# WesleyHsieh0806/TAO-Amodal

Measured on AMD Instinct MI355X. Metric: box-pair IoU+match throughput, higher is better.
Workload: dtype f64

## Files before the change

### include/tao_amodal_hip.h

```cpp
#ifndef TAO_AMODAL_HIP_H
#define TAO_AMODAL_HIP_H

#include <stddef.h>
#include <stdint.h>

#ifdef __cplusplus
extern "C" {
#endif

#define TAOAMD_N_THR 10
#define TAOAMD_N_REC 101
#define TAOAMD_LVIS_RNG 6
#define TAOAMD_TAO_RNG 20

#define TAOAMD_GT_IGNORE 1
#define TAOAMD_GT_OOF 2
#define TAOAMD_GT_ID_HIDDEN 4
#define TAOAMD_DT_IGNORE_UNMATCHED 1
#define TAOAMD_DT_NO_CONSUME 2

#define TAOAMD_OK 0
#define TAOAMD_ERR_HIP 1
#define TAOAMD_ERR_ARG 2
#define TAOAMD_ERR_TOO_LARGE 3
// ... 6 lines not shown

int taoamd_kernel_timing_enable(int on);
int taoamd_kernel_timing_label(const char *label);
int taoamd_kernel_timing_collect(char *names_host, size_t names_bytes,
                                 double *total_ms_host, int64_t *calls_host,
                                 int32_t max_kernels, int32_t *n_kernels_host);

int taoamd_thresholds_host(double *iou_thrs, double *rec_thrs);

int taoamd_set_thresholds(const double *iou_thrs, const double *rec_thrs);
int taoamd_set_ranges(const double *visibility_rng, const double *area_rng,
                      const double *time_rng);

int taoamd_bb_iou(const double *dt, const double *gt, size_t m, size_t n,
                  const unsigned char *iscrowd, double *o, void *stream);
int taoamd_bb_iou_host(const double *dt, const double *gt, size_t m, size_t n,
                       const unsigned char *iscrowd, double *o);

int taoamd_lvis_ranges(int64_t n_gt, const double *gt_vis,
                       const uint8_t *gt_flags, const int32_t *gt_cat,
                       const int32_t *gt_cat_off, int64_t n_dt,
                       const uint8_t *dt_flags, int32_t n_cat,
                       uint32_t *gt_rng, uint32_t *dt_rng, int32_t *num_gt,
                       void *stream);
int taoamd_tao_ranges(int64_t n_gt, const double *gt_area,
                      const int32_t *gt_len, const int32_t *gt_nhp,
                      const uint8_t *gt_flags, const int32_t *gt_cat,
                      const int32_t *gt_cat_off, int64_t n_dt,
                      const double *dt_area, const int32_t *dt_len,
                      const uint8_t *dt_flags, int32_t n_cat,
                      uint32_t *gt_rng, uint32_t *dt_rng, int32_t *num_gt,
                      void *stream);

size_t taoamd_rle_iou_workspace(int64_t n_dt, int64_t dt_total, int64_t n_gt,
                                int64_t gt_total);
int taoamd_rle_iou(int64_t n_cells, const int32_t *cell_dt_off,
                   const int32_t *cell_gt_off, const int64_t *cell_iou_off,
                   int64_t n_dt, int64_t dt_total, const int64_t *dt_off,
                   const uint32_t *dt_runs, const int32_t *dt_hw,
                   const double *dt_bb, int64_t n_gt, int64_t gt_total,
                   const int64_t *gt_off, const uint32_t *gt_runs,
                   const int32_t *gt_hw, const double *gt_bb, double *iou,
                   void *workspace, size_t workspace_bytes, void *stream);

size_t taoamd_track_mask_iou_workspace(int64_t dt_frames, int64_t dt_total,
                                       int64_t gt_frames, int64_t gt_total);
// ... 465 lines not shown
```

### tao_amodal_amd/_lib.py

```python
import ctypes as C
import os

HERE = os.path.dirname(os.path.abspath(__file__))
SO_PATH = os.environ.get("TAOAMD_LIBRARY") or os.path.join(HERE, "libtao_amodal_hip.so")

OK = 0
ERR_HIP, ERR_ARG, JSON_FALLBACK = 1, 2, 16
N_THR, N_REC = 10, 101
LVIS_RNG, TAO_RNG = 6, 20
MAX_GT_PER_CELL = 3072
SEGMENT_TILE = 2816
ERROR_TYPES_TILE = 256
TRACK_ERROR_TYPES_TILE = 16
ERROR_TYPES = ("TP", "IGNORED", "DUP", "LOC", "CLS", "BOTH", "BKG")
ERROR_IMPACT_CHUNK = 256
ERROR_FIXES = ("BASE", "CLS", "LOC", "BOTH", "DUP", "BKG", "MISS", "FP", "FN")
TRACK_ASSOCIATION_TILE = 64
TRACK_ASSOCIATION_VIS = 8
ASSOC_TRACK_COLUMNS = ("frames", "covered", "ids", "switches", "fragments", "primary",
                       "primary_frames")
ASSOC_CAT_COLUMNS = ("tracks", "frames", "covered", "ids", "switches", "fragments",
                     "mostly_tracked", "mostly_lost")
ASSOC_VIS_COLUMNS = ("frames", "covered", "primary")

_vp, _i64, _i32, _sz = C.c_void_p, C.c_int64, C.c_int32, C.c_size_t

SIGNATURES = {
    "taoamd_strerror": (C.c_char_p, [C.c_int]),
    "taoamd_last_error": (C.c_char_p, []),
    "taoamd_version": (C.c_int, []),
    "taoamd_thresholds_host": (C.c_int, [_vp, _vp]),
    "taoamd_set_thresholds": (C.c_int, [_vp, _vp]),
    "taoamd_set_ranges": (C.c_int, [_vp, _vp, _vp]),
    "taoamd_kernel_timing_enable": (C.c_int, [C.c_int]),
    "taoamd_kernel_timing_label": (C.c_int, [C.c_char_p]),
    "taoamd_kernel_timing_collect": (C.c_int, [_vp, _sz, _vp, _vp, _i32, _vp]),
    "taoamd_bb_iou": (C.c_int, [_vp, _vp, _sz, _sz, _vp, _vp, _vp]),
    "taoamd_bb_iou_host": (C.c_int, [_vp, _vp, _sz, _sz, _vp, _vp]),
    "taoamd_lvis_ranges": (C.c_int, [_i64, _vp, _vp, _vp, _vp, _i64, _vp,
                                     _i32, _vp, _vp, _vp, _vp]),
    "taoamd_tao_ranges": (C.c_int, [_i64, _vp, _vp, _vp, _vp, _vp, _vp, _i64,
                                    _vp, _vp, _vp, _i32, _vp, _vp, _vp, _vp]),
    "taoamd_sort_segments_workspace": (_sz, [_i64]),
    "taoamd_sort_segments": (C.c_int, [_i64, _i32, _vp, _vp, _i32, _i32, _vp,
                                       _vp, _vp, _vp, _vp, _sz, _vp]),
    "taoamd_sort_plan_host": (C.c_int, [_i32, _vp, _vp, _vp, _vp, _vp, _vp]),
    "taoamd_sort_sampled_workspace": (_sz, [_i64, _i64, _i32]),
    "taoamd_sort_sampled_cap_limit": (C.c_int, [_i32]),
    "taoamd_sort_sampled_notify": (C.c_int, [_vp]),
    "taoamd_event_create": (C.c_int, [_vp]),
    "taoamd_event_destroy": (C.c_int, [_vp]),
    "taoamd_stream_wait_event": (C.c_int, [_vp, _vp]),
    "taoamd_sort_sampled": (C.c_int, [_i64, _i32, _vp, _vp, _i32, _i32, _vp, _i32, _vp,
                                      _i32, _vp, _i32, _vp, _i32, _vp, _vp, _vp, _vp,
                                      _sz, _vp]),
    "taoamd_track_iou": (C.c_int, [_i64, _vp, _vp, _vp, _i64, _vp, _vp, _vp,
                                   _vp, _vp, _vp, _i32, _vp, _vp, _vp]),
    "taoamd_track_iou_single": (C.c_int, [_i64, _vp, _vp, _vp, _vp, _vp, _vp, _i32,
                                          _vp, _vp, _vp]),
    "taoamd_track_iou_planned": (C.c_int, [_i64, _vp, _vp, _vp, _vp, _vp, _vp, _vp,
                                           _i32, _vp, _vp, _i64, _vp, _vp]),
    "taoamd_track_stream": (C.c_int, [_i64, _vp, _vp, _vp, _vp, _vp, _vp, _vp]),
    "taoamd_json_pred_workspace": (_sz, [_sz]),
# ... 245 lines not shown
```

### tao_amodal_amd/csrc/accumulate.hip

```cpp
#include <atomic>
#include <cstdlib>
#include <cstring>

#include "common.hpp"
#include "transpose64.hpp"
#include "workspace.hpp"

using namespace taoamd;

#ifndef ACC_CH
#define ACC_CH 256
#endif
#ifndef ACC_INLINE_CHUNKS
#define ACC_INLINE_CHUNKS 64
#endif

struct AccArgs {
    int64_t n_dt;
    int32_t n_cat, n_rng, n_words, n_chunks_max;
    int32_t paired;
    int32_t wide;
    const int32_t *cat_off;
    const uint64_t *matched;
    const uint64_t *ignored;
// ... 1358 lines not shown
{
    AccArgs a;
    acc_layout(c, n_dt, n_cat, n_rng, a);
    val = c.take<double>(taoamd_compact_elems(n_cat, n_rng));
    rec = c.take<double>((size_t)n_cat * n_rng * N_THR);
}

extern "C" size_t taoamd_accumulate_workspace(int64_t n_dt, int32_t n_cat,
                                              int32_t n_rng)
{
    double *val, *rec;
    return measure([&](Carve &c) { acc_full_layout(c, n_dt, n_cat, n_rng, val, rec); });
}

enum { ACC_ALL = 0, ACC_PLAN = 1, ACC_SWEEP = 2 };

static int accumulate_compact(int64_t n_dt, int32_t n_cat, int32_t n_rng,
                              const int32_t *cat_off, const int32_t *order,
                              const uint64_t *matched, const uint64_t *ignored,
                              const int32_t *num_gt, int32_t k_begin, int32_t k_end,
                              int32_t max_segment, double *val, double *rec,
                              void *workspace, size_t workspace_bytes, void *stream,
                              int phase = ACC_ALL, int force_mode = SWEEP_AUTO,
                              const uint32_t *compact = nullptr)
{
    if (n_cat <= 0 || n_rng < 1 || n_rng > 32) return TAOAMD_ERR_ARG;
    if (k_begin < 0 || k_end > n_cat || k_begin > k_end) return TAOAMD_ERR_ARG;
    if (!cat_off || !workspace) return TAOAMD_ERR_ARG;
    if (phase != ACC_PLAN && (!num_gt || !val || !rec)) return TAOAMD_ERR_ARG;
    Carve c(workspace);
    AccArgs a;
    const AccWs t = acc_layout(c, n_dt, n_cat, n_rng, a);
    if (!c.fits(workspace, workspace_bytes)) return TAOAMD_ERR_WORKSPACE;
    if (k_begin == k_end) return TAOAMD_OK;
    hipStream_t s = (hipStream_t)stream;
    a.chunk_tab = nullptr;
    a.n_dt = n_dt; a.n_cat = n_cat; a.n_rng = n_rng;
    a.cat_off = cat_off; a.matched = matched; a.ignored = ignored; a.order = order;
    a.compact = compact;
    a.paired = matched != nullptr && ignored == matched + 1;
    a.wide = a.paired && ((uintptr_t)matched & 15) == 0;
    a.num_gt = num_gt; a.val = (uint64_t *)val; a.rec = rec;
    a.k_begin = k_begin; a.k_end = k_end;
    a.inline_scans = 0;
    a.sc_rows = 0; a.sc_gen = 0;
    a.sc_error = nullptr;
    a.sc_giveups = g_sweep_giveups.load(std::memory_order_relaxed);
// ... 35 lines not shown
    a.inline_scans = max_segment > 0 && max_segment <= ACC_INLINE_CHUNKS * ACC_CH;
    const size_t nc = (size_t)a.n_chunks_max, nw = (size_t)a.n_words;
    const int mode = force_mode != SWEEP_AUTO ? force_mode : sweep_mode(n_dt);
    if (compact != nullptr && (mode == SWEEP_CHUNKED || !order || !a.wide || a.n_words != 1 || n_rng > 6))
        return TAOAMD_ERR_ARG;
    if (mode != SWEEP_CHUNKED) {
        a.sc_rows = SWEEP_SW * SWEEP_NB * WAVE;
        a.inline_scans = 0;
    }
    if (mode != SWEEP_CHUNKED && max_segment > 0) a.xcd_start = t.xcd_start;
    if (phase == ACC_SWEEP) a.chunk_tab = t.chunk_tab;
    const unsigned chunk_blocks = (unsigned)((nc * nw + 3) / 4);
    const unsigned cat_blocks = (unsigned)((size_t)(k_end - k_begin) * nw);
    if (phase != ACC_SWEEP)
        TAO_TIMED("acc_chunks_kernel", s, acc_chunks_kernel<<<1, 256, 0, s>>>(a));
    if (phase == ACC_PLAN) {
        TAO_TIMED("acc_chunktab_kernel", s, acc_chunktab_kernel<<<(unsigned)((nc + 255) / 256), 256, 0, s>>>(a, t.chunk_tab));
        if (mode != SWEEP_CHUNKED)
            TAO_HIP(hipMemsetAsync(t.header, 0, t.head_bytes, s));
        TAO_LAUNCH_CHECK();
        return TAOAMD_OK;
    }
    if (mode != SWEEP_CHUNKED) {
        {
            const int64_t n_cj = (int64_t)n_cat * n_rng * N_REC;
            TAO_TIMED("acc_cj_kernel", s, acc_cj_kernel<<<(unsigned)((n_cj + 255) / 256), 256, 0, s>>>(a, rec_thr()));
        }
        const size_t n_sc = (size_t)(n_dt / a.sc_rows) + (size_t)n_cat + 1;
        const unsigned grid = a.xcd_start == nullptr
            ? (unsigned)(n_sc * nw)
            : (unsigned)(N_XCD * (n_sc / N_XCD + (size_t)max_segment / a.sc_rows + 3) * nw);
        if (mode == SWEEP_LOOKBACK) {
            if (phase == ACC_ALL)
                TAO_HIP(hipMemsetAsync(t.header, 0, t.head_bytes, s));
            uint32_t g = ++g_sc_gen;
            a.sc_gen = (g & 0x3fffffffu) ? (g & 0x3fffffffu) : (++g_sc_gen & 0x3fffffffu);
            a.sc_error = t.header;
            if (a.compact)
                TAO_TIMED("acc_sweep_kernel", s, (acc_sweep_kernel<SWEEP_SW, 0, 2><<<grid, SWEEP_SW * WAVE, 0, s>>>(a, rec_thr())));
            else if (a.order)
                TAO_TIMED("acc_sweep_kernel", s, (acc_sweep_kernel<SWEEP_SW, 0, 1><<<grid, SWEEP_SW * WAVE, 0, s>>>(a, rec_thr())));
            else
                TAO_TIMED("acc_sweep_kernel", s, (acc_sweep_kernel<SWEEP_SW, 0><<<grid, SWEEP_SW * WAVE, 0, s>>>(a, rec_thr())));
        } else if (a.compact) {
            TAO_TIMED("acc_sccount_kernel", s, (acc_sweep_kernel<SWEEP_SW, 2, 2><<<grid, SWEEP_SW * WAVE, 0, s>>>(a, rec_thr())));
            TAO_TIMED("acc_sweep_kernel", s, (acc_sweep_kernel<SWEEP_SW, 1, 2><<<grid, SWEEP_SW * WAVE, 0, s>>>(a, rec_thr())));
        } else if (a.order) {
// ... 15 lines not shown
    } else {
        TAO_TIMED("acc_prefix_kernel", s, acc_prefix_kernel<<<cat_blocks, 256, 0, s>>>(a, rec_thr()));
        TAO_TIMED("acc_chunkmax_kernel", s, acc_chunkmax_kernel<false><<<chunk_blocks, 256, 0, s>>>(a, rec_thr()));
        TAO_TIMED("acc_sufmax_kernel", s, acc_sufmax_kernel<<<cat_blocks, 256, 0, s>>>(a));
        TAO_TIMED("acc_emit_kernel", s, acc_emit_kernel<false><<<chunk_blocks, 256, 0, s>>>(a));
    }
    TAO_LAUNCH_CHECK();
    return TAOAMD_OK;
}

extern "C" int taoamd_accumulate_error(const void *workspace, void *stream, int32_t *flag_host)
{
    if (!workspace || !flag_host) return TAOAMD_ERR_ARG;
    Carve c((void *)workspace);
    AccArgs a;
    const uint32_t *w = acc_layout(c, 0, 1, 1, a).header;
    uint32_t f = 0;
    TAO_HIP(hipMemcpyAsync(&f, w, sizeof f, hipMemcpyDeviceToHost, (hipStream_t)stream));
    TAO_HIP(hipStreamSynchronize((hipStream_t)stream));
    *flag_host = (int32_t)f;
    return TAOAMD_OK;
}

extern "C" int taoamd_accumulate_compact(int64_t n_dt, int32_t n_cat,
                                         int32_t n_rng, const int32_t *cat_off,
                                         const uint64_t *matched,
                                         const uint64_t *ignored,
                                         const int32_t *num_gt, int32_t k_begin,
                                         int32_t k_end, int32_t max_segment,
                                         double *val, double *rec,
                                         void *workspace, size_t workspace_bytes,
                                         void *stream)
{
    return accumulate_compact(n_dt, n_cat, n_rng, cat_off, nullptr, matched, ignored,
                              num_gt, k_begin, k_end, max_segment, val, rec,
                              workspace, workspace_bytes, stream);
}

extern "C" int taoamd_finalize(int32_t n_cat, int32_t n_rng,
                               const int32_t *num_gt, const double *val,
                               const double *rec, double *precision,
                               double *recall, void *stream)
{
    if (n_cat <= 0 || n_rng < 1 || n_rng > 32) return TAOAMD_ERR_ARG;
    if (!num_gt || !val || !rec || !precision || !recall) return TAOAMD_ERR_ARG;
    FinArgs f;
    f.n_cat = n_cat; f.n_rng = n_rng; f.num_gt = num_gt; f.val = (const uint64_t *)val; f.rec = rec;
    f.precision = precision; f.recall = recall;
    const int64_t KR = (int64_t)n_cat * n_rng;
    dim3 grid((unsigned)((KR + FIN_RT - 1) / FIN_RT),
              (unsigned)((N_THR * N_REC + FIN_CT - 1) / FIN_CT));
    TAO_TIMED("acc_finalize_kernel", (hipStream_t)stream, acc_finalize_kernel<<<grid, 256, 0, (hipStream_t)stream>>>(f));
    TAO_LAUNCH_CHECK();
    return TAOAMD_OK;
}

static int accumulate_all(int64_t n_dt, int32_t n_cat, int32_t n_rng,
                          const int32_t *cat_off, const int32_t *order,
                          const uint64_t *matched, const uint64_t *ignored,
                          const int32_t *num_gt, int32_t max_segment,
                          double *precision, double *recall, void *workspace,
                          size_t workspace_bytes, void *stream, int phase = ACC_ALL,
                          int force_mode = SWEEP_AUTO, const uint32_t *compact = nullptr)
{
    if (n_cat <= 0 || n_rng < 1 || n_rng > 32) return TAOAMD_ERR_ARG;
    if (!workspace) return TAOAMD_ERR_ARG;
    Carve c(workspace);
    double *val, *rec;
    acc_full_layout(c, n_dt, n_cat, n_rng, val, rec);
    if (!c.fits(workspace, workspace_bytes)) return TAOAMD_ERR_WORKSPACE;
    int st = accumulate_compact(n_dt, n_cat, n_rng, cat_off, order, matched, ignored,
                                num_gt, 0, n_cat, max_segment, val, rec, workspace,
                                workspace_bytes, stream, phase, force_mode, compact);
    if (st != TAOAMD_OK || phase == ACC_PLAN) return st;
    return taoamd_finalize(n_cat, n_rng, num_gt, val, rec, precision, recall, stream);
}

extern "C" int taoamd_accumulate(int64_t n_dt, int32_t n_cat, int32_t n_rng,
                                 const int32_t *cat_off,
                                 const uint64_t *matched,
                                 const uint64_t *ignored, const int32_t *num_gt,
                                 int32_t max_segment, double *precision,
                                 double *recall, void *workspace,
                                 size_t workspace_bytes, void *stream)
{
    return accumulate_all(n_dt, n_cat, n_rng, cat_off, nullptr, matched, ignored,
                          num_gt, max_segment, precision, recall, workspace,
                          workspace_bytes, stream);
}

extern "C" int taoamd_accumulate_chunked(int64_t n_dt, int32_t n_cat, int32_t n_rng,
                                         const int32_t *cat_off,
                                         const uint64_t *matched,
                                         const uint64_t *ignored, const int32_t *num_gt,
                                         int32_t max_segment, double *precision,
                                         double *recall, void *workspace,
// ... 42 lines not shown
                                                   const uint64_t *ignored,
                                                   const int32_t *num_gt, int32_t max_segment,
                                                   double *precision, double *recall,
                                                   void *workspace, size_t workspace_bytes,
                                                   void *stream)
{
    if (!order) return TAOAMD_ERR_ARG;
    return accumulate_all(n_dt, n_cat, n_rng, cat_off, order, matched, ignored,
                          num_gt, max_segment, precision, recall, workspace,
                          workspace_bytes, stream, ACC_SWEEP);
}

extern "C" int taoamd_accumulate_by_order_compact(int64_t n_dt, int32_t n_cat, int32_t n_rng,
                                                  const int32_t *cat_off,
                                                  const int32_t *order,
                                                  const uint32_t *compact,
                                                  const uint64_t *rows,
                                                  const int32_t *num_gt, int32_t max_segment,
                                                  double *precision, double *recall,
                                                  void *workspace, size_t workspace_bytes,
                                                  int32_t prepared, void *stream)
{
    if (!order || !compact || !rows) return TAOAMD_ERR_ARG;
    return accumulate_all(n_dt, n_cat, n_rng, cat_off, order, rows, rows + 1,
                          num_gt, max_segment, precision, recall, workspace,
                          workspace_bytes, stream, prepared ? ACC_SWEEP : ACC_ALL,
                          SWEEP_AUTO, compact);
}

extern "C" int taoamd_accumulate_by_order_chunked(int64_t n_dt, int32_t n_cat, int32_t n_rng,
                                                  const int32_t *cat_off,
                                                  const int32_t *order,
                                                  const uint64_t *matched,
                                                  const uint64_t *ignored,
                                                  const int32_t *num_gt, int32_t max_segment,
                                                  double *precision, double *recall,
                                                  void *workspace, size_t workspace_bytes,
                                                  void *stream)
{
    if (!order) return TAOAMD_ERR_ARG;
    return accumulate_all(n_dt, n_cat, n_rng, cat_off, order, matched, ignored,
                          num_gt, max_segment, precision, recall, workspace,
                          workspace_bytes, stream, ACC_ALL, SWEEP_CHUNKED);
}

extern "C" int taoamd_accumulate_prepare(int64_t n_dt, int32_t n_cat, int32_t n_rng,
                                         const int32_t *cat_off, int32_t max_segment,
                                         void *workspace, size_t workspace_bytes,
                                         void *stream)
{
// ... 19 lines not shown
```

### tao_amodal_amd/csrc/common.hpp

```cpp
#pragma once
#include <hip/hip_runtime.h>
#include <stdint.h>

#include "../../include/tao_amodal_hip.h"

#define WAVE 64
#define N_THR TAOAMD_N_THR
#define N_REC TAOAMD_N_REC

struct IouThr {
    double v[N_THR];
};
struct RecThr {
    double v[N_REC];
};
struct RangeTab {
    double vis_lo[5], vis_hi[5];
    double area_lo[5], area_hi[5];
    double time_lo[4], time_hi[4];
};

namespace taoamd {

void set_error(hipError_t e, const char *what);
const IouThr &iou_thr();
const RecThr &rec_thr();
const RangeTab &range_tab();

#define TAO_HIP(call)                                     \
    do {                                                  \
        hipError_t e_ = (call);                           \
        if (e_ != hipSuccess) {                           \
            taoamd::set_error(e_, #call);                 \
            return TAOAMD_ERR_HIP;                        \
        }                                                 \
    } while (0)

extern bool g_timing_on;
void timing_begin(const char *name, hipStream_t s);
void timing_end(hipStream_t s);
struct KernelTimer {
    hipStream_t s;
    bool on;
    KernelTimer(const char *name, hipStream_t s_) : s(s_), on(g_timing_on)
    {
        if (on) timing_begin(name, s);
    }
    ~KernelTimer()
    {
        if (on) timing_end(s);
// ... 98 lines not shown
```

### tao_amodal_amd/csrc/iou_match.hip

```cpp
#include <cstdlib>

#include "common.hpp"

using namespace taoamd;

static IouThr match_thr()
{
    IouThr t = iou_thr();
    for (int q = 0; q < N_THR; q++) t.v[q] = t.v[q] < 1 - 1e-10 ? t.v[q] : 1 - 1e-10;
    return t;
}


__global__ void bb_iou_kernel(const double *__restrict__ dt,
                              const double *__restrict__ gt, size_t m,
                              size_t n, const unsigned char *__restrict__ crowd,
                              double *__restrict__ o)
{
    size_t total = m * n;
    for (size_t i = blockIdx.x * (size_t)blockDim.x + threadIdx.x; i < total;
         i += (size_t)gridDim.x * blockDim.x) {
        size_t g = i / m, d = i - g * m;
        const double4 D = reinterpret_cast<const double4 *>(dt)[d];
        const double4 G = reinterpret_cast<const double4 *>(gt)[g];
// ... 68 lines not shown
            }
        gt_rng[i] = m;
        if (num_gt != nullptr) {
            int32_t *row = num_gt + (int64_t)gcat[i] * TAOAMD_TAO_RNG;
            for (int r = 0; r < TAOAMD_TAO_RNG; r++)
                if (!((m >> r) & 1u)) atomicAdd(row + r, 1);
        }
    }
    if (i < n_dt) {
        uint32_t m = 0;
        bool nel = dflags[i] & TAOAMD_DT_IGNORE_UNMATCHED;
        double a_ = darea[i], len = (double)dlen[i];
#pragma unroll
        for (int a = 0; a < 5; a++)
#pragma unroll
            for (int t = 0; t < 4; t++)
                if (nel || a_ < alo[a] || a_ > ahi[a] || len < tlo[t] ||
                    len > thi[t])
                    m |= 1u << (a * 4 + t);
        dt_rng[i] = m;
    }
}

__global__ __launch_bounds__(256) void count_gt_kernel(
    int32_t n_cat, int32_t n_rng, const int32_t *__restrict__ gt_cat_off,
    const uint32_t *__restrict__ gt_rng, int32_t *__restrict__ num_gt)
{
    __shared__ int32_t part[4][32];
    const int wave = __builtin_amdgcn_readfirstlane(threadIdx.x >> 6);
    const int32_t k = blockIdx.x;
    const int lane = lane_id();
    const int32_t b = gt_cat_off[k], e = gt_cat_off[k + 1];
    int32_t mine = 0;
    for (int32_t base = b + wave * WAVE; base < e; base += 4 * 4 * WAVE) {
        uint32_t m[4];
#pragma unroll
        for (int u = 0; u < 4; u++) {
            const int32_t i = base + u * 4 * WAVE + lane;
            m[u] = i < e ? gt_rng[i] : 0xffffffffu;
        }
#pragma unroll
        for (int u = 0; u < 4; u++)
            for (int r = 0; r < n_rng; r++) {
                const int c = __popcll(__ballot(!((m[u] >> r) & 1u)));
                if (lane == r) mine += c;
            }
    }
    if (lane < 32) part[wave][lane] = mine;
    __syncthreads();
    if (threadIdx.x < (unsigned)n_rng)
        num_gt[(int64_t)k * n_rng + threadIdx.x] =
            part[0][threadIdx.x] + part[1][threadIdx.x] + part[2][threadIdx.x] +
            part[3][threadIdx.x];
}

struct MatchArgs {
    int64_t n_cells;
    const int32_t *cell_dt_off;
    const int32_t *cell_gt_off;
    const int64_t *cell_iou_off;
    const double *dt_box;
    const double *gt_box;
    const double *iou;
    const uint32_t *gt_rng;
    const uint32_t *dt_rng;
    const uint8_t *gt_flags;
    const uint8_t *dt_flags;
    const int32_t *dst;
    uint64_t *matched;
    uint64_t *ignored;
    int32_t *match_gt;
    double *ious_out;
    int32_t n_rng;
    int32_t n_words;
    int64_t out_stride;
    int32_t paired;
// ... 519 lines not shown

extern "C" int taoamd_lvis_ranges(int64_t n_gt, const double *gt_vis,
                                  const uint8_t *gt_flags,
                                  const int32_t *gt_cat,
                                  const int32_t *gt_cat_off, int64_t n_dt,
                                  const uint8_t *dt_flags, int32_t n_cat,
                                  uint32_t *gt_rng, uint32_t *dt_rng,
                                  int32_t *num_gt, void *stream)
{
    hipStream_t s = (hipStream_t)stream;
    const bool grouped = gt_cat_off != nullptr;
    if (!grouped)
        TAO_HIP(hipMemsetAsync(num_gt, 0, sizeof(int32_t) * (size_t)n_cat * TAOAMD_LVIS_RNG, s));
    if (dt_rng == nullptr) n_dt = 0;
    int64_t n = n_gt > n_dt ? n_gt : n_dt;
    if (n > 0) {
        TAO_TIMED("lvis_ranges_kernel", s, lvis_ranges_kernel<<<(unsigned)((n + 255) / 256), 256, 0, s>>>(
            n_gt, gt_vis, gt_flags, gt_cat, n_dt, dt_flags, gt_rng, dt_rng,
            grouped ? nullptr : num_gt, range_tab()));
    }
    if (grouped)
        TAO_TIMED("count_gt_kernel", s, count_gt_kernel<<<(unsigned)n_cat, 256, 0, s>>>(
            n_cat, TAOAMD_LVIS_RNG, gt_cat_off, gt_rng, num_gt));
    TAO_LAUNCH_CHECK();
    return TAOAMD_OK;
}

extern "C" int taoamd_tao_ranges(int64_t n_gt, const double *gt_area,
                                 const int32_t *gt_len, const int32_t *gt_nhp,
                                 const uint8_t *gt_flags, const int32_t *gt_cat,
                                 const int32_t *gt_cat_off, int64_t n_dt,
                                 const double *dt_area, const int32_t *dt_len,
                                 const uint8_t *dt_flags, int32_t n_cat,
                                 uint32_t *gt_rng, uint32_t *dt_rng,
                                 int32_t *num_gt, void *stream)
{
    hipStream_t s = (hipStream_t)stream;
    const bool grouped = gt_cat_off != nullptr;
    if (!grouped)
        TAO_HIP(hipMemsetAsync(num_gt, 0, sizeof(int32_t) * (size_t)n_cat * TAOAMD_TAO_RNG, s));
    int64_t n = n_gt > n_dt ? n_gt : n_dt;
    if (n > 0) {
        TAO_TIMED("tao_ranges_kernel", s, tao_ranges_kernel<<<(unsigned)((n + 255) / 256), 256, 0, s>>>(
            n_gt, gt_area, gt_len, gt_nhp, gt_flags, gt_cat, n_dt, dt_area,
            dt_len, dt_flags, gt_rng, dt_rng, grouped ? nullptr : num_gt, range_tab()));
    }
// ... 238 lines not shown
```

### tao_amodal_amd/csrc/sort.hip

```cpp
#include <algorithm>
#include <cstdlib>
#include <cstring>

#include "common.hpp"
#include "workspace.hpp"

using namespace taoamd;

#define RS_THREADS 256
#define RS_WAVES (RS_THREADS / WAVE)
#define RS_ITEMS 8
#define RS_TILE (RS_THREADS * RS_ITEMS)
#define RS_BINS 256
#define RS_PASSES 12

struct SortBufs {
    uint64_t *key[2];
    int32_t *idx[2];
    const int32_t *cat;
    uint32_t *block_hist;
    uint32_t *digit_total;
    int32_t *skip;
    int32_t *sel;
    int64_t n;
// ... 1149 lines not shown
        }
        if (k < 3) __syncthreads();
    }
    int32_t at[R];
    double ks[R];
#pragma unroll
    for (int r = 0; r < R; r++) {
        at[r] = c.begin + (int32_t)(v[r] & ((1u << SS_IDX_BITS) - 1));
        const int q = rank[r] + 1;
        if (v[r] == SS_PAD || q % S != 0 || q / S >= B) at[r] = -1;
    }
#pragma unroll
    for (int r = 0; r < R; r++) ks[r] = a.score[at[r] >= 0 ? at[r] : c.begin];
#pragma unroll
    for (int r = 0; r < R; r++) {
        if (at[r] >= 0) {
            const int q = rank[r] + 1;
            a.spl_key[c.bucket0 + q / S] = desc_key(ks[r]);
            a.spl_idx[c.bucket0 + q / S] = at[r];
        }
    }
}

__global__ __launch_bounds__(256) void ss_split4_kernel(SsArgs a, int32_t n_split)
{
    __shared__ uint64_t run[WAVE * 8];
    const int lane = lane_id();
    const int wave = __builtin_amdgcn_readfirstlane(threadIdx.x >> 6);
    const SsChunk c = a.chunks[a.split_list[blockIdx.x]];
    const int32_t m = ss_over(c.n) * c.n_buckets;
    if (m <= 256) ss_split_chunk4<1>(a, c, lane, wave, run);
    else if (m <= 512) ss_split_chunk4<2>(a, c, lane, wave, run);
    else if (m <= 1024) ss_split_chunk4<4>(a, c, lane, wave, run);
    else ss_split_chunk4<8>(a, c, lane, wave, run);
}

__global__ __launch_bounds__(256) void ss_split_kernel(SsArgs a, int32_t n_split)
{
    const int lane = lane_id();
    const int32_t w = (int32_t)blockIdx.x * 4 + (int32_t)(threadIdx.x >> 6);
    if (w >= n_split) return;
    const SsChunk c = a.chunks[a.split_list[w]];
    const int32_t m = ss_over(c.n) * c.n_buckets;
    if (m <= 128) ss_split_chunk<2>(a, c, lane);
    else if (m <= 256) ss_split_chunk<4>(a, c, lane);
    else if (m <= 512) ss_split_chunk<8>(a, c, lane);
    else if (m <= 1024) ss_split_chunk<16>(a, c, lane);
    else ss_split_chunk<32>(a, c, lane);
}

__global__ __launch_bounds__(SEG_THREADS) void ss_scatter_kernel(SsArgs a)
{
    __shared__ uint64_t s_key[SS_MAXB];
    __shared__ int32_t s_idx[SS_MAXB];
    __shared__ int32_t s_cnt[SS_MAXB], s_base[SS_MAXB];
    const uint32_t blk = xcd_block(blockIdx.x, gridDim.x);
    const SsChunk c = a.chunks[a.stile_chunk[blk]];
    const int32_t B = c.n_buckets;
    const int32_t t0 = c.begin + ((int32_t)blk - c.stile0) * SEG_TILE;
    const int32_t t1 = min(t0 + SEG_TILE, c.begin + c.n);
    if (threadIdx.x < SS_MAXB) {
// ... 314 lines not shown
                c.n_buckets = B; c.stile0 = (int32_t)nt; c.final = len <= SS_CHUNK;
                c.cat = k; c.pad = 0;
                memcpy(chunks + 8 * nc, &c, sizeof c);
                if (B > 1) split_list[ns] = (int32_t)nc;
                for (int32_t t = 0; t < tiles; t++) stile_chunk[nt + t] = (int32_t)nc;
                for (int32_t b = 0; b < B; b++) bucket_chunk[nb + b] = (int32_t)nc;
            }
            nc++;
            ns += B > 1;
            nt += tiles;
            nb += B;
        }
    }
    if (nb >= INT32_MAX / 2) return TAOAMD_ERR_TOO_LARGE;
    sizes[0] = nc; sizes[1] = ns; sizes[2] = nt; sizes[3] = nb; sizes[4] = merge;
    return TAOAMD_OK;
}

static size_t ss_layout(Carve &c, int64_t n, int64_t n_buckets, int merge, SsArgs &a, SegArgs &m)
{
    if (n < 1) n = 1;
    if (n_buckets < 1) n_buckets = 1;
    const size_t nb = (size_t)n_buckets;
    const size_t cursor_ints = align256((nb + 64) * 4) / 4;
    a.cursor = c.take<int32_t>(cursor_ints + nb);
    a.redo = Carve::at(a.cursor, cursor_ints);
    a.spl_key = c.take<uint64_t>(nb);
    a.spl_idx = c.take<int32_t>(nb);
    a.slot_key = c.take<uint64_t>(nb * SS_CAP);
    a.slot_idx = c.take<int32_t>(nb * SS_CAP);
    m.key[0] = m.key[1] = nullptr; m.idx[0] = m.idx[1] = nullptr; m.bnd = nullptr;
    if (merge) key_idx_layout(c, n, m);
    return cursor_ints;
}

extern "C" size_t taoamd_sort_sampled_workspace(int64_t n, int64_t n_buckets, int32_t merge)
{
    SsArgs a;
    SegArgs m;
    return measure([&](Carve &c) { ss_layout(c, n, n_buckets, merge, a, m); });
}

static thread_local hipEvent_t g_ss_notify = nullptr;
extern "C" int taoamd_sort_sampled_notify(void *event)
{
    g_ss_notify = (hipEvent_t)event;
    return TAOAMD_OK;
// ... 22 lines not shown
        return TAOAMD_ERR_ARG;
    const int merge = max_segment > SS_CHUNK;
    if (merge && (!tile_off || n_tiles <= 0)) return TAOAMD_ERR_ARG;
    Carve c(workspace);
    SsArgs a;
    SegArgs m;
    const size_t cursor_ints = ss_layout(c, n, n_buckets, merge, a, m);
    if (!c.fits(workspace, workspace_bytes)) return TAOAMD_ERR_WORKSPACE;
    hipStream_t s = (hipStream_t)stream;
    a.score = dt_score; a.chunks = (const SsChunk *)chunks; a.split_list = split_list;
    a.stile_chunk = stile_chunk; a.bucket_chunk = bucket_chunk;
    a.order = order; a.dst = dst; a.n_buckets = n_buckets; a.n_stiles = n_stiles;
    a.cap_limit = g_ss_cap_limit;
#ifdef TAOAMD_ABLATE
    static const int dbg_env = getenv("TAOAMD_SS_DBG") ? atoi(getenv("TAOAMD_SS_DBG")) : 0;
    a.dbg = dbg_env;
#else
    a.dbg = 0;
#endif
    m.cat_off = cat_off; m.tile_off = tile_off; m.cat = nullptr; m.score = dt_score;
    m.order = order; m.dst = dst; m.n = n; m.n_cat = n_cat; m.n_tiles = n_tiles;
    a.key_out = m.key[SS_FIRST_MERGE_PASS & 1];
    a.idx_out = m.idx[SS_FIRST_MERGE_PASS & 1];
    TAO_HIP(hipMemsetAsync(a.cursor, 0, cursor_ints * 4, s));
    if (n_split > 0) {
        static const bool one_wave = getenv("TAOAMD_SS_SPLIT") && atoi(getenv("TAOAMD_SS_SPLIT")) == 1;
        if (one_wave)
            TAO_TIMED("ss_split_kernel", s, ss_split_kernel<<<(unsigned)((n_split + 3) / 4), 256, 0, s>>>(a, n_split));
        else
            TAO_TIMED("ss_split_kernel", s, ss_split4_kernel<<<(unsigned)n_split, 256, 0, s>>>(a, n_split));
        if (g_ss_notify) TAO_HIP(hipEventRecord(g_ss_notify, s));
        TAO_TIMED("ss_scatter_kernel", s, ss_scatter_kernel<<<(unsigned)n_stiles, SEG_THREADS, 0, s>>>(a));
    } else if (g_ss_notify) {
        TAO_HIP(hipEventRecord(g_ss_notify, s));
    }
    g_ss_notify = nullptr;
    TAO_TIMED("ss_sort_kernel", s, ss_sort_kernel<<<(unsigned)((n_buckets + 3) / 4), 256, 0, s>>>(a));
    TAO_TIMED("ss_redo_kernel", s, ss_redo_kernel<<<(unsigned)std::min<int64_t>(1024, (n_buckets + 3) / 4), 256, 0, s>>>(a));
    if (merge) {
        int passes = 0;
        for (int64_t L = SEG_TILE; L < max_segment; L <<= 1) passes++;
        for (int p = SS_FIRST_MERGE_PASS; p < passes; p++)
            TAO_TIMED("seg_mpass_kernel", s, seg_mpass_kernel<<<(unsigned)n_tiles, 256, 0, s>>>(m, p, p == passes - 1, SS_CHUNK));
    }
    TAO_LAUNCH_CHECK();
    return TAOAMD_OK;
}
```

### tao_amodal_amd/engine.py

```python
import os

import numpy as np
import torch

from . import _lib

N_THR, N_REC = _lib.N_THR, _lib.N_REC


def _ptr(t):
    return None if t is None else t.data_ptr()


def _stream():
    return torch.cuda.current_stream().cuda_stream


def _to_device(v, device):
    from .flatten import LazyRows
    if not isinstance(v, LazyRows):
        return torch.from_numpy(np.ascontiguousarray(v)).to(device)
    from .flatten_dev import device_copy
    src = device_copy(v.source, device)
    if len(v.index) == 0:
# ... 447 lines not shown
    return out


Workspace.order = property(_order_of)


def expand_rows(ws):
    if ws.rows_pending:
        dp = ws._dp
        with torch.cuda.device(dp.device):
            _lib.check(_lib.load().taoamd_expand_rows(
                dp.n_dt, dp.n_rng, _ptr(ws.compact_buf), _ptr(ws._rows), _stream()),
                "taoamd_expand_rows")
        ws.rows_pending = False
        ws.rows_expanded += 1
    return ws


Workspace.rows = property(lambda ws: expand_rows(ws)._rows)
Workspace.matched = property(lambda ws: expand_rows(ws)._matched)
Workspace.ignored = property(lambda ws: expand_rows(ws)._ignored)


def stage_ranges(dp, ws):
    lib, t, s = _lib.load(), dp.t, _stream()
    if dp.kind == "lvis":
        _lib.check(lib.taoamd_lvis_ranges(
            dp.n_gt, _ptr(t["gt_vis"]), _ptr(t["gt_flags"]), _ptr(t["gt_cat"]),
            _ptr(t["gt_cat_off"]) if dp.grouped else None,
            dp.n_dt, _ptr(t["dt_flags"]), dp.n_cat, _ptr(ws.gt_rng),
            _ptr(ws.dt_rng), _ptr(ws.num_gt), s), "taoamd_lvis_ranges")
    else:
        _lib.check(lib.taoamd_tao_ranges(
            dp.n_gt, _ptr(t["gt_area"]), _ptr(t["gt_len"]), _ptr(t["gt_nhp"]),
            _ptr(t["gt_flags"]), _ptr(t["gt_cat"]),
            _ptr(t["gt_cat_off"]) if dp.grouped else None, dp.n_dt,
            _ptr(t["dt_area"]), _ptr(t["dt_len"]), _ptr(t["dt_flags"]),
            dp.n_cat, _ptr(ws.gt_rng), _ptr(ws.dt_rng), _ptr(ws.num_gt), s),
            "taoamd_tao_ranges")


import os as _os0
SORT_SAMPLED_MIN = 1_500_000
_SORT_FORCE = _os0.environ.get("TAOAMD_SORT", "")


def sort_is_sampled(dp):
    if _SORT_FORCE in ("sampled", "segments"):
        return _SORT_FORCE == "sampled"
# ... 285 lines not shown
            _ptr(t["dt_box"]), _ptr(t["gt_box"]), dp.n_rng, _ptr(ws.gt_rng),
            _ptr(t["gt_flags"]), _ptr(t["dt_flags"]), _ptr(ws._rows), _ptr(ws.compact_buf),
            _ptr(t["dt_group"]), _ptr(t["dt_meta"]), g_ptr, n_g, s_ptr, n_s, s),
            "taoamd_match_compact")
        ws.rows_pending = True
        return
    if groups is None:
        ws.rows_pending = False
    _lib.check(lib.taoamd_match(
        dp.n_cells, _ptr(t["cell_dt_off"]), _ptr(t["cell_gt_off"]),
        _ptr(t["cell_iou_off"]), dp.max_g,
        _ptr(t["dt_box"]) if fused else None,
        _ptr(t["gt_box"]) if fused else None,
        None if fused else _ptr(ws.iou), dp.n_rng, _ptr(ws.gt_rng),
        None if dp.kind == "lvis" else _ptr(ws.dt_rng),
        _ptr(t["gt_flags"]), _ptr(t["dt_flags"]),
        _ptr(ws.dst) if scatter else None, 0, _ptr(ws.matched),
        _ptr(ws.ignored), _ptr(ws.match_gt if match_gt is None else match_gt),
        _ptr(ws.ious_out),
        _ptr(t["dt_group"]), _ptr(t["dt_meta"]), g_ptr, n_g,
        s_ptr, n_s, s), "taoamd_match")


def stage_accumulate_by_order(dp, ws):
    lib, t, s = _lib.load(), dp.t, _stream()
    key = _plan_key(dp)
    if ws.rows_pending and key[1] in (2, 3):
        _lib.check(lib.taoamd_accumulate_by_order_compact(
            dp.n_dt, dp.n_cat, dp.n_rng, _ptr(t["cat_off"]), _ptr(ws.order),
            _ptr(ws.compact_buf), _ptr(ws._rows), _ptr(ws.num_gt), dp.acc_hint,
            _ptr(ws.precision), _ptr(ws.recall), _ptr(ws.acc_ws), ws.acc_bytes,
            int(ws.acc_prepared == key), s), "taoamd_accumulate_by_order_compact")
        return
    fn = lib.taoamd_accumulate_by_order_prepared if ws.acc_prepared == key \
        else lib.taoamd_accumulate_by_order
    _lib.check(fn(
        dp.n_dt, dp.n_cat, dp.n_rng, _ptr(t["cat_off"]), _ptr(ws.order),
        _ptr(ws.matched), _ptr(ws.ignored), _ptr(ws.num_gt), dp.acc_hint,
        _ptr(ws.precision), _ptr(ws.recall), _ptr(ws.acc_ws), ws.acc_bytes, s),
        "taoamd_accumulate_by_order")


def stage_accumulate(dp, ws):
    lib, t, s = _lib.load(), dp.t, _stream()
    fn = lib.taoamd_accumulate_prepared if ws.acc_prepared == _plan_key(dp) \
        else lib.taoamd_accumulate
    _lib.check(fn(
        dp.n_dt, dp.n_cat, dp.n_rng, _ptr(t["cat_off"]), _ptr(ws.matched),
        _ptr(ws.ignored), _ptr(ws.num_gt), dp.acc_hint, _ptr(ws.precision),
        _ptr(ws.recall), _ptr(ws.acc_ws), ws.acc_bytes, s),
        "taoamd_accumulate")


def stage_scores(dp, ws):
    lib, t, s = _lib.load(), dp.t, _stream()
# ... 328 lines not shown
    def wrap(self, name, fn, dp, ws):
        a = torch.cuda.Event(enable_timing=True)
        b = torch.cuda.Event(enable_timing=True)
        a.record()
        fn(dp, ws)
        b.record()
        self.events.setdefault(name, []).append((a, b))

    def mean_ms(self):
        return {k: sum(a.elapsed_time(b) for a, b in v) / len(v)
                for k, v in self.events.items()}


PROBE = None


def _probed(name, fn, dp, ws):
    if PROBE is None:
        fn(dp, ws)
    else:
        PROBE.wrap(dp.kind + ":" + name, fn, dp, ws)


def run_forked(dp, ws, aux, head_only=False, sort_aside=None, no_match=False,
               sort_done=None, match_done=None):
    cur = torch.cuda.current_stream(dp.device)
    aux.wait_stream(cur)
    if _lib.TIMING:
        _lib.kernel_timing_label(dp.kind)
    if sort_aside is None:
        sort_aside = ws.gather and _plan_key(dp)[1] in (2, 3)
    if sort_aside and dp.kind == "lvis" and not dp.mask_iou and not head_only \
            and not no_match and dp.grouped and dp.n_dt:
        order_only = sort_is_sampled(dp) and ws.order_buf is not None
        if order_only and not ws.dst_identity:
            torch.arange(dp.n_dt, out=ws.dst[:dp.n_dt])
            ws.dst_identity = True
        with torch.cuda.stream(aux):
            stage_sort(dp, ws, order_only=order_only)
            if sort_done is not None:
                sort_done.record(aux)
        stage_ranges(dp, ws)
        _probed("match", lambda d, w: stage_match(d, w, scatter=False), dp, ws)
        if match_done is not None:
            match_done.record(cur)
        cur.wait_stream(aux)
        stage_accumulate_by_order(dp, ws)
        return
    if dp.kind == "lvis":
        with torch.cuda.stream(aux):
            stage_ranges(dp, ws)
            stage_mask_iou(dp, ws)
        stage_sort(dp, ws)
        if sort_done is not None:
            sort_done.record(cur)
    else:
        with torch.cuda.stream(aux):
            stage_ranges(dp, ws)
            stage_sort(dp, ws)
        _probed("track_iou", stage_track_iou_guarded, dp, ws)
        if dp.guard_flat is not None:
            ws.guarded_pairs = apply_iou_guard(dp, ws)
    cur.wait_stream(aux)
    if no_match:
        return
    _probed("match", stage_match, dp, ws)
    if match_done is not None:
        match_done.record(cur)
    if not head_only:
        stage_accumulate(dp, ws)
# ... 75 lines not shown
```

Before: 47230.

## Fold recall-crossing table into GT counting and cursor zeroing into split kernel

Adds a ranges variant whose per-category GT counting kernel also fills the accumulator's recall-crossing (cj) table, so the later accumulate call can skip its separate acc_cj_kernel launch. The engine enables this on the forked LVIS path when the accumulator plan is already prepared. Separately, the sampled sort drops its hipMemsetAsync of the bucket cursor and instead appends extra workgroups to the split kernel that zero it. Both changes aim to remove small launches and memset overhead from the critical path, at the cost of more coupling between stages through the shared workspace layout.

```diff
diff --git a/include/tao_amodal_hip.h b/include/tao_amodal_hip.h
--- a/include/tao_amodal_hip.h
+++ b/include/tao_amodal_hip.h
@@ -52,6 +52,13 @@
                        const int32_t *gt_cat_off, int64_t n_dt,
                        const uint8_t *dt_flags, int32_t n_cat,
                        uint32_t *gt_rng, uint32_t *dt_rng, int32_t *num_gt,
+                       void *stream);
+int taoamd_lvis_ranges_crossings(int64_t n_gt, const double *gt_vis,
+                       const uint8_t *gt_flags, const int32_t *gt_cat,
+                       const int32_t *gt_cat_off, int64_t n_dt,
+                       const uint8_t *dt_flags, int32_t n_cat,
+                       uint32_t *gt_rng, uint32_t *dt_rng, int32_t *num_gt,
+                       void *acc_workspace, size_t acc_workspace_bytes,
                        void *stream);
 int taoamd_tao_ranges(int64_t n_gt, const double *gt_area,
                       const int32_t *gt_len, const int32_t *gt_nhp,
diff --git a/tao_amodal_amd/_lib.py b/tao_amodal_amd/_lib.py
--- a/tao_amodal_amd/_lib.py
+++ b/tao_amodal_amd/_lib.py
@@ -39,6 +39,8 @@
     "taoamd_bb_iou_host": (C.c_int, [_vp, _vp, _sz, _sz, _vp, _vp]),
     "taoamd_lvis_ranges": (C.c_int, [_i64, _vp, _vp, _vp, _vp, _i64, _vp,
                                      _i32, _vp, _vp, _vp, _vp]),
+    "taoamd_lvis_ranges_crossings": (C.c_int, [_i64, _vp, _vp, _vp, _vp, _i64, _vp,
+                                               _i32, _vp, _vp, _vp, _vp, _sz, _vp]),
     "taoamd_tao_ranges": (C.c_int, [_i64, _vp, _vp, _vp, _vp, _vp, _vp, _i64,
                                     _vp, _vp, _vp, _i32, _vp, _vp, _vp, _vp]),
     "taoamd_sort_segments_workspace": (_sz, [_i64]),
diff --git a/tao_amodal_amd/csrc/accumulate.hip b/tao_amodal_amd/csrc/accumulate.hip
--- a/tao_amodal_amd/csrc/accumulate.hip
+++ b/tao_amodal_amd/csrc/accumulate.hip
@@ -1404,7 +1404,7 @@
                               int32_t max_segment, double *val, double *rec,
                               void *workspace, size_t workspace_bytes, void *stream,
                               int phase = ACC_ALL, int force_mode = SWEEP_AUTO,
-                              const uint32_t *compact = nullptr)
+                              const uint32_t *compact = nullptr, bool cj_ready = false)
 {
     if (n_cat <= 0 || n_rng < 1 || n_rng > 32) return TAOAMD_ERR_ARG;
     if (k_begin < 0 || k_end > n_cat || k_begin > k_end) return TAOAMD_ERR_ARG;
@@ -1486,7 +1486,7 @@
         return TAOAMD_OK;
     }
     if (mode != SWEEP_CHUNKED) {
-        {
+        if (!cj_ready) {
             const int64_t n_cj = (int64_t)n_cat * n_rng * N_REC;
             TAO_TIMED("acc_cj_kernel", s, acc_cj_kernel<<<(unsigned)((n_cj + 255) / 256), 256, 0, s>>>(a, rec_thr()));
         }
@@ -1548,6 +1548,18 @@
     return TAOAMD_OK;
 }
 
+int32_t *taoamd::acc_cj_table(void *workspace, size_t workspace_bytes, int64_t n_dt,
+                              int32_t n_cat, int32_t n_rng)
+{
+    Carve c(workspace);
+    AccArgs a;
+    acc_layout(c, n_dt, n_cat, n_rng, a);
+    double *val, *rec;
+    Carve full(workspace);
+    acc_full_layout(full, n_dt, n_cat, n_rng, val, rec);
+    return full.fits(workspace, workspace_bytes) ? a.cj : nullptr;
+}
+
 extern "C" int taoamd_accumulate_compact(int64_t n_dt, int32_t n_cat,
                                          int32_t n_rng, const int32_t *cat_off,
                                          const uint64_t *matched,
@@ -1587,7 +1599,8 @@
                           const int32_t *num_gt, int32_t max_segment,
                           double *precision, double *recall, void *workspace,
                           size_t workspace_bytes, void *stream, int phase = ACC_ALL,
-                          int force_mode = SWEEP_AUTO, const uint32_t *compact = nullptr)
+                          int force_mode = SWEEP_AUTO, const uint32_t *compact = nullptr,
+                          bool cj_ready = false)
 {
     if (n_cat <= 0 || n_rng < 1 || n_rng > 32) return TAOAMD_ERR_ARG;
     if (!workspace) return TAOAMD_ERR_ARG;
@@ -1597,7 +1610,7 @@
     if (!c.fits(workspace, workspace_bytes)) return TAOAMD_ERR_WORKSPACE;
     int st = accumulate_compact(n_dt, n_cat, n_rng, cat_off, order, matched, ignored,
                                 num_gt, 0, n_cat, max_segment, val, rec, workspace,
-                                workspace_bytes, stream, phase, force_mode, compact);
+                                workspace_bytes, stream, phase, force_mode, compact, cj_ready);
     if (st != TAOAMD_OK || phase == ACC_PLAN) return st;
     return taoamd_finalize(n_cat, n_rng, num_gt, val, rec, precision, recall, stream);
 }
@@ -1686,10 +1699,11 @@
                                                   int32_t prepared, void *stream)
 {
     if (!order || !compact || !rows) return TAOAMD_ERR_ARG;
+    if (prepared < 0 || prepared > 3 || prepared == 2) return TAOAMD_ERR_ARG;
     return accumulate_all(n_dt, n_cat, n_rng, cat_off, order, rows, rows + 1,
                           num_gt, max_segment, precision, recall, workspace,
                           workspace_bytes, stream, prepared ? ACC_SWEEP : ACC_ALL,
-                          SWEEP_AUTO, compact);
+                          SWEEP_AUTO, compact, (prepared & 2) != 0);
 }
 
 extern "C" int taoamd_accumulate_by_order_chunked(int64_t n_dt, int32_t n_cat, int32_t n_rng,
diff --git a/tao_amodal_amd/csrc/common.hpp b/tao_amodal_amd/csrc/common.hpp
--- a/tao_amodal_amd/csrc/common.hpp
+++ b/tao_amodal_amd/csrc/common.hpp
@@ -26,6 +26,8 @@
 const IouThr &iou_thr();
 const RecThr &rec_thr();
 const RangeTab &range_tab();
+int32_t *acc_cj_table(void *workspace, size_t workspace_bytes, int64_t n_dt,
+                      int32_t n_cat, int32_t n_rng);
 
 #define TAO_HIP(call)                                     \
     do {                                                  \
diff --git a/tao_amodal_amd/csrc/iou_match.hip b/tao_amodal_amd/csrc/iou_match.hip
--- a/tao_amodal_amd/csrc/iou_match.hip
+++ b/tao_amodal_amd/csrc/iou_match.hip
@@ -114,11 +114,10 @@
     }
 }
 
-__global__ __launch_bounds__(256) void count_gt_kernel(
-    int32_t n_cat, int32_t n_rng, const int32_t *__restrict__ gt_cat_off,
-    const uint32_t *__restrict__ gt_rng, int32_t *__restrict__ num_gt)
-{
-    __shared__ int32_t part[4][32];
+__device__ __forceinline__ int32_t count_gt_category(
+    int32_t n_rng, const int32_t *__restrict__ gt_cat_off,
+    const uint32_t *__restrict__ gt_rng, int32_t *__restrict__ num_gt, int32_t (*part)[32])
+{
     const int wave = __builtin_amdgcn_readfirstlane(threadIdx.x >> 6);
     const int32_t k = blockIdx.x;
     const int lane = lane_id();
@@ -140,10 +139,39 @@
     }
     if (lane < 32) part[wave][lane] = mine;
     __syncthreads();
-    if (threadIdx.x < (unsigned)n_rng)
-        num_gt[(int64_t)k * n_rng + threadIdx.x] =
-            part[0][threadIdx.x] + part[1][threadIdx.x] + part[2][threadIdx.x] +
-            part[3][threadIdx.x];
+    int32_t total = 0;
+    if (threadIdx.x < (unsigned)n_rng) {
+        total = part[0][threadIdx.x] + part[1][threadIdx.x] + part[2][threadIdx.x] +
+                part[3][threadIdx.x];
+        num_gt[(int64_t)k * n_rng + threadIdx.x] = total;
+    }
+    return total;
+}
+
+__global__ __launch_bounds__(256) void count_gt_kernel(
+    int32_t n_cat, int32_t n_rng, const int32_t *__restrict__ gt_cat_off,
+    const uint32_t *__restrict__ gt_rng, int32_t *__restrict__ num_gt)
+{
+    __shared__ int32_t part[4][32];
+    count_gt_category(n_rng, gt_cat_off, gt_rng, num_gt, part);
+}
+
+__global__ __launch_bounds__(256) void count_gt_cj_kernel(
+    int32_t n_cat, int32_t n_rng, const int32_t *__restrict__ gt_cat_off,
+    const uint32_t *__restrict__ gt_rng, int32_t *__restrict__ num_gt,
+    int32_t *__restrict__ cj, RecThr rec)
+{
+    __shared__ int32_t part[4][32];
+    __shared__ int32_t total[32];
+    const int32_t t = count_gt_category(n_rng, gt_cat_off, gt_rng, num_gt, part);
+    if (threadIdx.x < (unsigned)n_rng) total[threadIdx.x] = t;
+    __syncthreads();
+    int32_t *row = cj + (int64_t)blockIdx.x * n_rng * N_REC;
+    for (int32_t i = threadIdx.x; i < n_rng * N_REC; i += 256) {
+        const int32_t r = i / N_REC;
+        const int32_t ng = total[r];
+        row[i] = ng > 0 ? recall_crossing(rec.v[i - r * N_REC], ng) : 0;
+    }
 }
 
 struct MatchArgs {
@@ -709,6 +737,32 @@
     if (grouped)
         TAO_TIMED("count_gt_kernel", s, count_gt_kernel<<<(unsigned)n_cat, 256, 0, s>>>(
             n_cat, TAOAMD_LVIS_RNG, gt_cat_off, gt_rng, num_gt));
+    TAO_LAUNCH_CHECK();
+    return TAOAMD_OK;
+}
+
+extern "C" int taoamd_lvis_ranges_crossings(int64_t n_gt, const double *gt_vis,
+                                            const uint8_t *gt_flags,
+                                            const int32_t *gt_cat,
+                                            const int32_t *gt_cat_off, int64_t n_dt,
+                                            const uint8_t *dt_flags, int32_t n_cat,
+                                            uint32_t *gt_rng, uint32_t *dt_rng,
+                                            int32_t *num_gt, void *acc_workspace,
+                                            size_t acc_workspace_bytes, void *stream)
+{
+    if (!gt_cat_off || !num_gt || !acc_workspace || n_cat <= 0 || n_dt < 0)
+        return TAOAMD_ERR_ARG;
+    int32_t *cj = acc_cj_table(acc_workspace, acc_workspace_bytes, n_dt, n_cat, TAOAMD_LVIS_RNG);
+    if (!cj) return TAOAMD_ERR_WORKSPACE;
+    hipStream_t s = (hipStream_t)stream;
+    if (dt_rng == nullptr) n_dt = 0;
+    int64_t n = n_gt > n_dt ? n_gt : n_dt;
+    if (n > 0) {
+        TAO_TIMED("lvis_ranges_kernel", s, lvis_ranges_kernel<<<(unsigned)((n + 255) / 256), 256, 0, s>>>(
+            n_gt, gt_vis, gt_flags, gt_cat, n_dt, dt_flags, gt_rng, dt_rng, nullptr, range_tab()));
+    }
+    TAO_TIMED("count_gt_kernel", s, count_gt_cj_kernel<<<(unsigned)n_cat, 256, 0, s>>>(
+        n_cat, TAOAMD_LVIS_RNG, gt_cat_off, gt_rng, num_gt, cj, rec_thr()));
     TAO_LAUNCH_CHECK();
     return TAOAMD_OK;
 }
diff --git a/tao_amodal_amd/csrc/sort.hip b/tao_amodal_amd/csrc/sort.hip
--- a/tao_amodal_amd/csrc/sort.hip
+++ b/tao_amodal_amd/csrc/sort.hip
@@ -1195,14 +1195,41 @@
     }
 }
 
+#define SS_ZERO_PER 16
+#define SS_ZERO_WGS_MAX 64
+
+__host__ __device__ inline int64_t ss_cursor_ints(int64_t n_buckets)
+{
+    return ((n_buckets + 64) * 4 + 255) / 256 * 64;
+}
+
+__device__ __forceinline__ void ss_zero_cursor(const SsArgs &a, int32_t first_wg)
+{
+    const int32_t n_zero = (int32_t)ss_cursor_ints(a.n_buckets);
+    const int32_t stride = (int32_t)(gridDim.x - first_wg) * (int32_t)blockDim.x;
+    for (int32_t i = (int32_t)(blockIdx.x - first_wg) * (int32_t)blockDim.x + (int32_t)threadIdx.x;
+         i < n_zero; i += stride)
+        a.cursor[i] = 0;
+}
+
+static unsigned ss_zero_wgs(size_t n_zero)
+{
+    return (unsigned)std::min<size_t>((n_zero + 256 * SS_ZERO_PER - 1) / (256 * SS_ZERO_PER),
+                                      SS_ZERO_WGS_MAX);
+}
+
 __global__ __launch_bounds__(256) void ss_split4_kernel(SsArgs a, int32_t n_split)
 {
     __shared__ uint64_t run[WAVE * 8];
     const int lane = lane_id();
     const int wave = __builtin_amdgcn_readfirstlane(threadIdx.x >> 6);
-    const SsChunk c = a.chunks[a.split_list[blockIdx.x]];
-    const int32_t m = ss_over(c.n) * c.n_buckets;
-    if (m <= 256) ss_split_chunk4<1>(a, c, lane, wave, run);
+    const bool zeroing = (int32_t)blockIdx.x >= n_split;
+    const SsChunk c = a.chunks[a.split_list[zeroing ? 0 : blockIdx.x]];
+    const int32_t m = zeroing ? 0 : ss_over(c.n) * c.n_buckets;
+    if (m <= 256) {
+        if (m == 0) ss_zero_cursor(a, n_split);
+        else ss_split_chunk4<1>(a, c, lane, wave, run);
+    }
     else if (m <= 512) ss_split_chunk4<2>(a, c, lane, wave, run);
     else if (m <= 1024) ss_split_chunk4<4>(a, c, lane, wave, run);
     else ss_split_chunk4<8>(a, c, lane, wave, run);
@@ -1210,6 +1237,11 @@
 
 __global__ __launch_bounds__(256) void ss_split_kernel(SsArgs a, int32_t n_split)
 {
+    const int32_t n_wgs = (n_split + 3) / 4;
+    if ((int32_t)blockIdx.x >= n_wgs) {
+        ss_zero_cursor(a, n_wgs);
+        return;
+    }
     const int lane = lane_id();
     const int32_t w = (int32_t)blockIdx.x * 4 + (int32_t)(threadIdx.x >> 6);
     if (w >= n_split) return;
@@ -1570,7 +1602,7 @@
     if (n < 1) n = 1;
     if (n_buckets < 1) n_buckets = 1;
     const size_t nb = (size_t)n_buckets;
-    const size_t cursor_ints = align256((nb + 64) * 4) / 4;
+    const size_t cursor_ints = (size_t)ss_cursor_ints((int64_t)nb);
     a.cursor = c.take<int32_t>(cursor_ints + nb);
     a.redo = Carve::at(a.cursor, cursor_ints);
     a.spl_key = c.take<uint64_t>(nb);
@@ -1639,17 +1671,20 @@
     m.order = order; m.dst = dst; m.n = n; m.n_cat = n_cat; m.n_tiles = n_tiles;
     a.key_out = m.key[SS_FIRST_MERGE_PASS & 1];
     a.idx_out = m.idx[SS_FIRST_MERGE_PASS & 1];
-    TAO_HIP(hipMemsetAsync(a.cursor, 0, cursor_ints * 4, s));
     if (n_split > 0) {
+        if (n_buckets < 2) return TAOAMD_ERR_ARG;
+        if (cursor_ints > (size_t)INT32_MAX) return TAOAMD_ERR_TOO_LARGE;
+        const unsigned zero_wgs = ss_zero_wgs(cursor_ints);
         static const bool one_wave = getenv("TAOAMD_SS_SPLIT") && atoi(getenv("TAOAMD_SS_SPLIT")) == 1;
         if (one_wave)
-            TAO_TIMED("ss_split_kernel", s, ss_split_kernel<<<(unsigned)((n_split + 3) / 4), 256, 0, s>>>(a, n_split));
+            TAO_TIMED("ss_split_kernel", s, ss_split_kernel<<<(unsigned)((n_split + 3) / 4) + zero_wgs, 256, 0, s>>>(a, n_split));
         else
-            TAO_TIMED("ss_split_kernel", s, ss_split4_kernel<<<(unsigned)n_split, 256, 0, s>>>(a, n_split));
+            TAO_TIMED("ss_split_kernel", s, ss_split4_kernel<<<(unsigned)n_split + zero_wgs, 256, 0, s>>>(a, n_split));
         if (g_ss_notify) TAO_HIP(hipEventRecord(g_ss_notify, s));
         TAO_TIMED("ss_scatter_kernel", s, ss_scatter_kernel<<<(unsigned)n_stiles, SEG_THREADS, 0, s>>>(a));
-    } else if (g_ss_notify) {
-        TAO_HIP(hipEventRecord(g_ss_notify, s));
+    } else {
+        TAO_HIP(hipMemsetAsync(a.cursor, 0, cursor_ints * 4, s));
+        if (g_ss_notify) TAO_HIP(hipEventRecord(g_ss_notify, s));
     }
     g_ss_notify = nullptr;
     TAO_TIMED("ss_sort_kernel", s, ss_sort_kernel<<<(unsigned)((n_buckets + 3) / 4), 256, 0, s>>>(a));
diff --git a/tao_amodal_amd/engine.py b/tao_amodal_amd/engine.py
--- a/tao_amodal_amd/engine.py
+++ b/tao_amodal_amd/engine.py
@@ -493,9 +493,15 @@
 Workspace.ignored = property(lambda ws: expand_rows(ws)._ignored)
 
 
-def stage_ranges(dp, ws):
+def stage_ranges(dp, ws, crossings=False):
     lib, t, s = _lib.load(), dp.t, _stream()
-    if dp.kind == "lvis":
+    if crossings:
+        _lib.check(lib.taoamd_lvis_ranges_crossings(
+            dp.n_gt, _ptr(t["gt_vis"]), _ptr(t["gt_flags"]), _ptr(t["gt_cat"]),
+            _ptr(t["gt_cat_off"]), dp.n_dt, _ptr(t["dt_flags"]), dp.n_cat, _ptr(ws.gt_rng),
+            _ptr(ws.dt_rng), _ptr(ws.num_gt), _ptr(ws.acc_ws), ws.acc_bytes, s),
+            "taoamd_lvis_ranges_crossings")
+    elif dp.kind == "lvis":
         _lib.check(lib.taoamd_lvis_ranges(
             dp.n_gt, _ptr(t["gt_vis"]), _ptr(t["gt_flags"]), _ptr(t["gt_cat"]),
             _ptr(t["gt_cat_off"]) if dp.grouped else None,
@@ -827,15 +833,18 @@
         s_ptr, n_s, s), "taoamd_match")
 
 
-def stage_accumulate_by_order(dp, ws):
+def stage_accumulate_by_order(dp, ws, crossings=False):
     lib, t, s = _lib.load(), dp.t, _stream()
     key = _plan_key(dp)
     if ws.rows_pending and key[1] in (2, 3):
+        prepared = int(ws.acc_prepared == key)
+        if crossings and prepared:
+            prepared |= 2
         _lib.check(lib.taoamd_accumulate_by_order_compact(
             dp.n_dt, dp.n_cat, dp.n_rng, _ptr(t["cat_off"]), _ptr(ws.order),
             _ptr(ws.compact_buf), _ptr(ws._rows), _ptr(ws.num_gt), dp.acc_hint,
             _ptr(ws.precision), _ptr(ws.recall), _ptr(ws.acc_ws), ws.acc_bytes,
-            int(ws.acc_prepared == key), s), "taoamd_accumulate_by_order_compact")
+            prepared, s), "taoamd_accumulate_by_order_compact")
         return
     fn = lib.taoamd_accumulate_by_order_prepared if ws.acc_prepared == key \
         else lib.taoamd_accumulate_by_order
@@ -1210,6 +1219,12 @@
         PROBE.wrap(dp.kind + ":" + name, fn, dp, ws)
 
 
+def _early_crossings(dp, ws):
+    key = _plan_key(dp)
+    return bool(ws.gather and ws.match_gt is None and ws.ious_out is None
+                and key[1] in (2, 3) and ws.acc_prepared == key)
+
+
 def run_forked(dp, ws, aux, head_only=False, sort_aside=None, no_match=False,
                sort_done=None, match_done=None):
     cur = torch.cuda.current_stream(dp.device)
@@ -1228,12 +1243,13 @@
             stage_sort(dp, ws, order_only=order_only)
             if sort_done is not None:
                 sort_done.record(aux)
-        stage_ranges(dp, ws)
+        crossings = _early_crossings(dp, ws)
+        stage_ranges(dp, ws, crossings=crossings)
         _probed("match", lambda d, w: stage_match(d, w, scatter=False), dp, ws)
         if match_done is not None:
             match_done.record(cur)
         cur.wait_stream(aux)
-        stage_accumulate_by_order(dp, ws)
+        stage_accumulate_by_order(dp, ws, crossings=crossings)
         return
     if dp.kind == "lvis":
         with torch.cuda.stream(aux):
```

New measurement: 47550, median of 6. No clear change (+0.7%).
